# zhangmozhe/Deep-Exemplar-based-Video-Colorization

Hardware: AMD Instinct MI355X
Metric: colorized frames/sec/GPU at 216x384; correlation HBM GB/s vs roofline (higher is better)
Workload: dtype f32

## Files before the change

deep-exemplar-based-video-colorization_amd/csrc/conv_mfma.hip:

```cpp
#include "conv_kernel.h"
#include "conv_sk_kernel.h"
#include <algorithm>

#include "conv_wino_kernel.h"

static int virt_dim(int S, int up, int sub) {
    if (up == 2) return S * 2;
    if (sub == 2) return (S + 1) / 2;
    return S;
}

extern "C" int dvc_conv2d_out_hw(const DvcConvDesc* d, int32_t* OH, int32_t* OW) {
    DVC_REQUIRE(d, "dvc_conv2d_out_hw: null descriptor");
    int VH = virt_dim(d->H, d->in_up, d->in_sub), VW = virt_dim(d->W, d->in_up, d->in_sub);
    int ext = d->dil * (d->ksize - 1) + 1;
    *OH = (VH + 2 * d->pad - ext) / d->stride + 1;
    *OW = (VW + 2 * d->pad - ext) / d->stride + 1;
    return 0;
}

static int pick_tw(int OW) {
    int best = 32, best_w = cdiv(OW, 32) * 32;
    for (int tw : {16, 8}) {
        int wpad = cdiv(OW, tw) * tw;
// ... 758 lines not shown
#pragma unroll
    for (int o = 0; o < COUT; ++o) {
        float v = ((part[0][o][px] + part[1][o][px]) + (part[2][o][px] + part[3][o][px])) + (bias ? bias[o] : 0.f);
        y[((long)n * COUT + o) * HW + p] = apply_act(v, act, 0.f);
    }
}

extern "C" int dvc_conv1x1_small(const float* x, const float* w, const float* bias, int32_t N,
                                 int32_t Cin, int32_t HW, int32_t Cout, int32_t act, float* y,
                                 dvcStream stream) {
    DVC_REQUIRE(x && w && y, "dvc_conv1x1_small: null argument");
    DVC_REQUIRE(Cout >= 1 && Cout <= 4, "dvc_conv1x1_small: Cout must be 1..4");
    dim3 grid(cdiv(HW, 64), N);
    hipStream_t s = (hipStream_t)stream;
    switch (Cout) {
        case 1: hipLaunchKernelGGL(conv1x1_small_kernel<1>, grid, dim3(256), 0, s, x, w, bias, Cin, (long)HW, act, y); break;
        case 2: hipLaunchKernelGGL(conv1x1_small_kernel<2>, grid, dim3(256), 0, s, x, w, bias, Cin, (long)HW, act, y); break;
        case 3: hipLaunchKernelGGL(conv1x1_small_kernel<3>, grid, dim3(256), 0, s, x, w, bias, Cin, (long)HW, act, y); break;
        default: hipLaunchKernelGGL(conv1x1_small_kernel<4>, grid, dim3(256), 0, s, x, w, bias, Cin, (long)HW, act, y); break;
    }
    DVC_CHECK_LAUNCH("dvc_conv1x1_small");
    return 0;
}
```

deep-exemplar-based-video-colorization_amd/csrc/conv_wino_kernel.h:

```cpp
#pragma once
#include <type_traits>

#include "conv_kernel.h"

typedef float f32x4 __attribute__((ext_vector_type(4)));
typedef float f32x2 __attribute__((ext_vector_type(2)));

struct ConvWinoArgs {
    ConvKArgs k;
    int ss;
    int blk_y, blk_x;
    int gx, gy, gz;
    unsigned m_gx, m_gxy, m_cls, m_blkx, m_split;
    const float* x2;
    long x2_bs;
    int cinA, H2, W2, VH2, VW2, in_up2, in_sub2;
    float* pool;
    long pool_bs;
};
__host__ __device__ __forceinline__ unsigned wino_magic(long d) {
    return d > 1 ? (unsigned)(((1ULL << 32) + (unsigned long long)d - 1) / (unsigned long long)d) : 0u;
}
__device__ __forceinline__ int wino_div(int n, unsigned magic) { return magic ? (int)__umulhi((unsigned)n, magic) : n; }

// ... 41 lines not shown
#define WINO_S_ADD(D, A, B) asm volatile("v_add_f32 %0, %1, %2" : "=v"(D) : "v"(A), "v"(B))
#define WINO_S_SUB(D, A, B) asm volatile("v_sub_f32 %0, %1, %2" : "=v"(D) : "v"(A), "v"(B))

__device__ __forceinline__ int wino_stored_offset(int VH, int VW, int W, int in_up, int in_sub, int pad_mode, int vy, int vx) {
    int sy = map_virtual(vy, VH, pad_mode);
    int sx = map_virtual(vx, VW, pad_mode);
    if (sy < 0 || sx < 0) return -1;
    if (in_up == 2) {
        sy >>= 1;
        sx >>= 1;
    } else if (in_sub == 2) {
        sy <<= 1;
        sx <<= 1;
    }
    return sy * W + sx;
}

#define WINO_NBUF 3
__host__ __device__ constexpr int wino_xs_floats(int wm, int wn, int tr, int kc) {
    return ((kc * (2 * tr * wn + 2) * wino_pitch(tr) + 128 * wm * wn - 1) / (128 * wm * wn)) * (128 * wm * wn);
}
__host__ __device__ constexpr int wino_us_floats(int wm, int kc) { return wm * kc * 128 * 4; }

template <int WM, int WN, int TR, int KC, int VAR = 0, bool DUAL = false, class SA = ConvWinoArgs, bool UPZ = false>
__device__ __forceinline__ void conv_wino_body(const SA& s, const int wlog, float* const xsb, float* const usb) {
#if defined(__HIP_DEVICE_COMPILE__)
    const auto& a = s.k;
    constexpr int NPAIR = WM * WN;
    constexpr int NT = 128 * NPAIR;
    constexpr int TC = 32 / TR;
    constexpr int PR = 2 * TR * WN + 2;
    constexpr int PC = 2 * TC + 2;
    constexpr int PITCH = wino_pitch(TR);
    constexpr int plane = PR * PITCH;
    constexpr int EPT = (KC * plane + NT - 1) / NT;
    constexpr int C_XS = EPT * NT;
    static_assert(C_XS == wino_xs_floats(WM, WN, TR, KC), "LDS size helper out of step");
    constexpr int UQ = WM * KC * 128;
    static_assert(UQ * 4 == wino_us_floats(WM, KC), "LDS size helper out of step");
    static_assert(UQ % NT == 0, "whole staging instructions");
    static_assert(PITCH >= PC && PITCH % 2 == 0 && plane % 2 == 0 && KC % 4 == 0, "aligned patch rows, even K-steps per chunk");
    static_assert(2 * (PITCH / 2) + 1 < 256, "ds_read2_b64 offsets are 8 bits");
    constexpr int WPT = UQ / NT;
    constexpr int NI = EPT + WPT;
    static_assert(2 * NI < 64, "vmcnt is 6 bits");
    constexpr int KS = KC / 2;
    constexpr int NBUF = WINO_NBUF;
    constexpr int OOB = (int)0x80000000;
    static_assert(!UPZ || DUAL, "the zero-position form is built for the two-input launches");
    static_assert(NBUF * UQ * 4 >= 2 * NPAIR * 32 * 64, "the output exchange fits in the filter buffers");

    const int tid = threadIdx.x;
    const int lane = tid & 63, wave = __builtin_amdgcn_readfirstlane(tid >> 6);
    const int l31 = lane & 31, hi = lane >> 5;
    const int ph = wave / NPAIR, pair = wave % NPAIR;
    const int wm = pair / WN, wn = pair % WN;
    const int tr = l31 / TC, tc = l31 % TC;
    const int ss = s.ss;
    const int bz = wino_div(wlog, s.m_gxy), r_xy = wlog - bz * (s.gx * s.gy);
    const int by = wino_div(r_xy, s.m_gx), bx = r_xy - by * s.gx;
    const int per_cls = s.blk_y * s.blk_x;
    const int cls = wino_div(bx, s.m_cls), brem = bx - cls * per_cls;
    const int py = ss == 2 ? cls >> 1 : 0, px = ss == 2 ? cls & 1 : 0;
    const int tyb = wino_div(brem, s.m_blkx);
    const int ty0 = tyb * (TR * WN), tx0 = (brem - tyb * s.blk_x) * TC;
    const int b0 = by * WM;
    const int n = wino_div(bz, s.m_split), ksplit = bz - n * a.split;
    const int HWi = a.H * a.W;

    const int nchunks_all = a.Cin / KC;
    const int c_begin = ksplit * a.chunks_per_split;
    const int c_end = min(nchunks_all, c_begin + a.chunks_per_split);

// ... 68 lines not shown
    constexpr std::false_type ANY_INPUT{};

    const unsigned xlane =
        (unsigned)(size_t)(CONV_AS3 float*)xsb + (hi * plane + (2 * (wn * TR + tr) + ph) * PITCH + 2 * tc) * 4;
    const unsigned ulane = (unsigned)(size_t)(CONV_AS3 float*)usb + (((wm * KC + hi) * 4 + 2 * ph) * 32 + l31) * 16;

    constexpr bool BRANCH_FREE = VAR != 3;
    issue_x(c_begin, 0, ANY_INPUT);
    if (BRANCH_FREE) {
        issue(min(c_begin + 1, c_end - 1), 1, ANY_INPUT);
        issue(min(c_begin + 2, c_end - 1), 2, ANY_INPUT);
        asm volatile("s_waitcnt vmcnt(%0)" ::"n"(2 * NI) : "memory");
    } else {
        if (c_begin + 1 < c_end) issue(c_begin + 1, 1, ANY_INPUT);
        if (c_begin + 2 < c_end) issue(c_begin + 2, 2, ANY_INPUT);
        if (c_begin + 2 < c_end) asm volatile("s_waitcnt vmcnt(%0)" ::"n"(2 * NI) : "memory");
        else if (c_begin + 1 < c_end) asm volatile("s_waitcnt vmcnt(%0)" ::"n"(NI) : "memory");
        else asm volatile("s_waitcnt vmcnt(0)" ::: "memory");
    }
    __builtin_amdgcn_s_barrier();

    const float slope = a.act_slope_ptr ? *a.act_slope_ptr : a.act_slope;
    const long OHW = (long)a.OH * a.OW;
    const bool partial = a.split > 1;
    float* yb = partial ? a.part + ((long)ksplit * a.N + n) * a.Cout * OHW : a.y + (long)n * a.y_bs;
    const float* rb = (!partial && a.res) ? a.res + (long)n * a.res_bs : nullptr;

    auto run = [&](auto PHC) {
        constexpr int PH = decltype(PHC)::value;
        f32x4 D[2][3], U[2][2];
        f32x2 V03[2][2], V12[2][2];
        auto lo = [](const f32x4& v) { return __builtin_shufflevector(v, v, 0, 1); };
        auto hh = [](const f32x4& v) { return __builtin_shufflevector(v, v, 2, 3); };
        auto transform_a = [&](const f32x4 (&d)[3], f32x2 (&tl)[2], f32x2 (&th)[2], const bool row3_only = false) {
            if (VAR == 1) {
                if (PH == 0) {
                    WINO_S_SUB(tl[0].x, d[0].x, d[2].x); WINO_S_SUB(tl[0].y, d[0].y, d[2].y);
                    WINO_S_SUB(th[0].x, d[0].z, d[2].z); WINO_S_SUB(th[0].y, d[0].w, d[2].w);
                    WINO_S_ADD(tl[1].x, d[1].x, d[2].x); WINO_S_ADD(tl[1].y, d[1].y, d[2].y);
                    WINO_S_ADD(th[1].x, d[1].z, d[2].z); WINO_S_ADD(th[1].y, d[1].w, d[2].w);
                } else {
                    if (!row3_only) {
                        WINO_S_SUB(tl[0].x, d[1].x, d[0].x); WINO_S_SUB(tl[0].y, d[1].y, d[0].y);
                        WINO_S_SUB(th[0].x, d[1].z, d[0].z); WINO_S_SUB(th[0].y, d[1].w, d[0].w);
                    }
                    WINO_S_SUB(tl[1].x, d[0].x, d[2].x); WINO_S_SUB(tl[1].y, d[0].y, d[2].y);
                    WINO_S_SUB(th[1].x, d[0].z, d[2].z); WINO_S_SUB(th[1].y, d[0].w, d[2].w);
// ... 110 lines not shown
                    s1[j] = -m[j] - m[4 + j];
                }
            }
            o[0] = s0[0] + s0[1] + s0[2];
            o[1] = s0[1] - s0[2] - s0[3];
            o[2] = s1[0] + s1[1] + s1[2];
            o[3] = s1[1] - s1[2] - s1[3];
        };
        auto for8 = [&](auto f) {
            f(std::integral_constant<int, 0>{}); f(std::integral_constant<int, 1>{}); f(std::integral_constant<int, 2>{});
            f(std::integral_constant<int, 3>{}); f(std::integral_constant<int, 4>{}); f(std::integral_constant<int, 5>{});
            f(std::integral_constant<int, 6>{}); f(std::integral_constant<int, 7>{});
        };
        {
            float* mine = ex + (wave * 32) * 64 + lane;
            for8([&](auto IC) {
                constexpr int i = decltype(IC)::value;
                float o[4];
                partial_out(std::integral_constant<int, 8 * (1 - PH) + i>{}, o);
#pragma unroll
                for (int q = 0; q < 4; ++q) mine[(i * 4 + q) * 64] = o[q];
            });
        }
        __syncthreads();
        const float* theirs = ex + ((PH == 0 ? wave + NPAIR : wave - NPAIR) * 32) * 64 + lane;
        const int u0 = 2 * (ty0 + wn * TR + tr), x0 = 2 * (tx0 + tc);
        const int oy0 = ss * u0 + py, oy1 = ss * (u0 + 1) + py;
        const int ox0 = ss * x0 + px, ox1 = ss * (x0 + 1) + px;
        const bool okx0 = ox0 < a.OW, okx1 = ox1 < a.OW;
        const bool pairst = ss == 1 && okx1 && (a.OW & 1) == 0;
        const bool pool_here = !partial && s.pool;
        float* pb = pool_here ? s.pool + (long)n * s.pool_bs : nullptr;
        const long PHW = (long)(a.OH >> 1) * (a.OW >> 1);
        for8([&](auto IC) {
            constexpr int i = decltype(IC)::value;
            constexpr int r = 8 * PH + i;
            float o[4];
            partial_out(std::integral_constant<int, r>{}, o);
#pragma unroll
            for (int q = 0; q < 4; ++q) {
                const float t = theirs[(i * 4 + q) * 64];
                o[q] = PH == 0 ? o[q] + t : t + o[q];
            }
            const int co = (b0 + wm) * 32 + (r & 3) + 8 * (r >> 2) + 4 * hi;
            const float bias = (!partial && a.bias) ? a.bias[co] : 0.f;
            float pooled = 0.f;
#pragma unroll
            for (int p = 0; p < 2; ++p) {
                const int oy = p ? oy1 : oy0;
                if (oy >= a.OH) continue;
                const long row = (long)co * OHW + (long)oy * a.OW;
                float v0 = o[2 * p] + bias, v1 = o[2 * p + 1] + bias;
                if (rb) {
                    if (okx0) v0 += rb[row + ox0];
                    if (okx1) v1 += rb[row + ox1];
                }
                if (!partial) {
                    v0 = apply_act(v0, a.act, slope);
                    v1 = apply_act(v1, a.act, slope);
                }
                if (pool_here) {
                    const float m = fmaxf(v0, v1);
                    pooled = p ? fmaxf(pooled, m) : m;
                    if (p && okx1) pb[(long)co * PHW + (long)(oy0 >> 1) * (a.OW >> 1) + (ox0 >> 1)] = pooled;
                    if (!a.y) continue;
                }
                if (pairst && VAR == 2) {
                    union { float2 f; unsigned long long u; } cv;
                    cv.f = make_float2(v0, v1);
                    __hip_atomic_store(reinterpret_cast<unsigned long long*>(yb + row + ox0), cv.u, __ATOMIC_RELAXED, __HIP_MEMORY_SCOPE_AGENT);
                } else if (pairst) {
                    *reinterpret_cast<float2*>(yb + row + ox0) = make_float2(v0, v1);
                } else {
                    if (okx0) yb[row + ox0] = v0;
                    if (okx1) yb[row + ox1] = v1;
                }
            }
        });
    };
    if (ph) run(std::integral_constant<int, 1>{});
    else run(std::integral_constant<int, 0>{});
#endif
}

template <int WM, int WN, int TR, int KC, int VAR = 0, bool DUAL = false, bool UPZ = false>
__global__ __launch_bounds__(128 * WM * WN) __attribute__((amdgpu_waves_per_eu(2, 2))) void conv_wino_kernel(ConvWinoArgs s) {
    __shared__ __attribute__((aligned(16))) float xsb[WINO_NBUF * wino_xs_floats(WM, WN, TR, KC)];
    __shared__ __attribute__((aligned(16))) float usb[WINO_NBUF * wino_us_floats(WM, KC)];
    const int G = s.gx * s.gy * s.gz;
    const int xq = G / 8, xr = G % 8, xcd = blockIdx.x % 8, xi = blockIdx.x / 8;
    const int wlog = (xcd < xr ? xcd * (xq + 1) : xr * (xq + 1) + (xcd - xr) * xq) + xi;
    conv_wino_body<WM, WN, TR, KC, VAR, DUAL, ConvWinoArgs, UPZ>(s, wlog, xsb, usb);
}

#define WINO_GROUP_MAX 4
struct ConvWinoGroupArgs {
    ConvWinoArgs item[WINO_GROUP_MAX];
    int per_xcd[WINO_GROUP_MAX + 1];
    int tr[WINO_GROUP_MAX];
    int n;
};
typedef __attribute__((address_space(4))) ConvWinoArgs ConvWinoArgsK;
template <int WM, int WN, int KC>
__global__ __launch_bounds__(128 * WM * WN) __attribute__((amdgpu_waves_per_eu(2, 2))) void conv_wino_group_kernel(ConvWinoGroupArgs g) {
    constexpr int XS = wino_xs_floats(WM, WN, 1, KC) > wino_xs_floats(WM, WN, 8, KC) ? wino_xs_floats(WM, WN, 1, KC) : wino_xs_floats(WM, WN, 8, KC);
    static_assert(XS >= wino_xs_floats(WM, WN, 2, KC) && XS >= wino_xs_floats(WM, WN, 4, KC), "largest patch buffer");
#if defined(__HIP_DEVICE_COMPILE__)
    __shared__ __attribute__((aligned(16))) float xsb[WINO_NBUF * XS];
    __shared__ __attribute__((aligned(16))) float usb[WINO_NBUF * wino_us_floats(WM, KC)];
    const int xcd = blockIdx.x % 8, xi = blockIdx.x / 8;
    int it = 0, base = 0, q = g.per_xcd[1], tr = g.tr[0];
#pragma unroll
    for (int i = 1; i < WINO_GROUP_MAX; ++i)
        if (i < g.n && xi >= g.per_xcd[i]) {
            it = i;
// ... 56 lines not shown
}

template <int WM, int WN, int KC>
static void conv_wino_launch_shape_dual(int tr, bool upz, dim3 grid, hipStream_t st, const ConvWinoArgs& s) {
    constexpr int NT = 128 * WM * WN;
    if (upz) {
        switch (tr) {
            case 1: hipLaunchKernelGGL((conv_wino_kernel<WM, WN, 1, KC, 0, true, true>), grid, dim3(NT), 0, st, s); break;
            case 2: hipLaunchKernelGGL((conv_wino_kernel<WM, WN, 2, KC, 0, true, true>), grid, dim3(NT), 0, st, s); break;
            case 4: hipLaunchKernelGGL((conv_wino_kernel<WM, WN, 4, KC, 0, true, true>), grid, dim3(NT), 0, st, s); break;
            default: hipLaunchKernelGGL((conv_wino_kernel<WM, WN, 8, KC, 0, true, true>), grid, dim3(NT), 0, st, s); break;
        }
        return;
    }
    switch (tr) {
        case 1: hipLaunchKernelGGL((conv_wino_kernel<WM, WN, 1, KC, 0, true>), grid, dim3(NT), 0, st, s); break;
        case 2: hipLaunchKernelGGL((conv_wino_kernel<WM, WN, 2, KC, 0, true>), grid, dim3(NT), 0, st, s); break;
        case 4: hipLaunchKernelGGL((conv_wino_kernel<WM, WN, 4, KC, 0, true>), grid, dim3(NT), 0, st, s); break;
        default: hipLaunchKernelGGL((conv_wino_kernel<WM, WN, 8, KC, 0, true>), grid, dim3(NT), 0, st, s); break;
    }
}

void conv_wino_launch_m1_dual(int tr, bool upz, dim3 grid, hipStream_t st, const ConvWinoArgs& s);
void conv_wino_launch_m4(int tr, dim3 grid, hipStream_t st, const ConvWinoArgs& s);
void conv_wino_launch_m2(int tr, dim3 grid, hipStream_t st, const ConvWinoArgs& s);
void conv_wino_launch_m1(int tr, dim3 grid, hipStream_t st, const ConvWinoArgs& s);
void conv_wino_launch_m0(int tr, dim3 grid, hipStream_t st, const ConvWinoArgs& s);
void conv_wino_launch_group_m1(dim3 grid, hipStream_t st, const ConvWinoGroupArgs& g);
```

deep-exemplar-based-video-colorization_amd/csrc/conv_wino_m1.hip:

```cpp
#include "conv_wino_kernel.h"

void conv_wino_launch_m1(int tr, dim3 grid, hipStream_t st, const ConvWinoArgs& s) {
    conv_wino_launch_shape<2, 1, 4>(tr, grid, st, s);
}

void conv_wino_launch_m1_dual(int tr, bool upz, dim3 grid, hipStream_t st, const ConvWinoArgs& s) {
    conv_wino_launch_shape_dual<2, 1, 4>(tr, upz, grid, st, s);
}
```

deep-exemplar-based-video-colorization_amd/dvc_amd/_lib.py:

```python
import ctypes
import os

_HERE = os.path.dirname(os.path.abspath(__file__))
DEBUG_BUILD = os.environ.get("DVC_DEBUG_LIB", "0") == "1"
LIB_PATH = os.path.join(_HERE, "libdvc_hip_debug.so" if DEBUG_BUILD else "libdvc_hip.so")
ABI_VERSION = 20

c_float_p = ctypes.c_void_p
c_i32 = ctypes.c_int32
c_i64 = ctypes.c_int64


class DvcConvDesc(ctypes.Structure):
    _fields_ = [
        ("N", c_i32), ("Cin", c_i32), ("H", c_i32), ("W", c_i32),
        ("Cout", c_i32), ("ksize", c_i32), ("stride", c_i32), ("dil", c_i32),
        ("pad", c_i32), ("pad_mode", c_i32), ("in_up", c_i32), ("in_sub", c_i32),
        ("act", c_i32), ("act_slope", ctypes.c_float), ("in_prelu", c_i32), ("cfg", c_i32), ("split_k", c_i32),
        ("x_batch_stride", c_i64), ("y_batch_stride", c_i64), ("res_batch_stride", c_i64),
        ("flags", c_i32), ("w_batch_stride", c_i64),
    ]


class DvcConvGroupItem(ctypes.Structure):
# ... 17 lines not shown
_VP = ctypes.c_void_p
SIGNATURES = {
    "dvc_abi_version": (ctypes.c_int, []),
    "dvc_last_error": (ctypes.c_char_p, []),
    "dvc_conv2d_out_hw": (ctypes.c_int, [ctypes.POINTER(DvcConvDesc), ctypes.POINTER(c_i32), ctypes.POINTER(c_i32)]),
    "dvc_conv2d": (ctypes.c_int, [ctypes.POINTER(DvcConvDesc), _VP, _VP, _VP, _VP, _VP, _VP, _VP, _VP, _VP, _VP,
                                  ctypes.c_size_t, _VP]),
    "dvc_winograd_weight_floats": (ctypes.c_size_t, [c_i32, c_i32]),
    "dvc_winograd_pack_weight": (ctypes.c_int, [_VP, c_i32, c_i32, _VP, _VP]),
    "dvc_conv2d_winograd_split": (ctypes.c_int, [ctypes.POINTER(DvcConvDesc), ctypes.c_size_t, ctypes.POINTER(c_i32),
                                                ctypes.POINTER(c_i32)]),
    "dvc_conv2d_winograd": (ctypes.c_int, [ctypes.POINTER(DvcConvDesc), _VP, _VP, _VP, _VP, _VP, _VP, _VP,
                                           ctypes.c_size_t, _VP]),
    "dvc_conv2d_winograd_pool": (ctypes.c_int, [ctypes.POINTER(DvcConvDesc), _VP, _VP, _VP, _VP, _VP, _VP, c_i64, _VP,
                                                ctypes.c_size_t, _VP]),
    "dvc_conv2d_winograd_dual": (ctypes.c_int, [ctypes.POINTER(DvcConvDesc), ctypes.POINTER(DvcConvDesc), _VP, _VP, _VP, _VP, _VP,
                                                _VP, _VP, ctypes.c_size_t, _VP]),
    "dvc_conv2d_ws_eligible": (ctypes.c_int, [ctypes.POINTER(DvcConvDesc)]),
    "dvc_conv2d_ws_pack_weight": (ctypes.c_int, [_VP, c_i32, c_i32, _VP, _VP]),
    "dvc_conv2d_ws": (ctypes.c_int, [ctypes.POINTER(DvcConvDesc), _VP, _VP, _VP, _VP, _VP, _VP]),
    "dvc_conv2d_winograd_group": (ctypes.c_int, [ctypes.POINTER(DvcConvGroupItem), c_i32, _VP]),
    "dvc_instnorm_apply_group": (ctypes.c_int, [ctypes.POINTER(DvcInstNormItem), c_i32, _VP]),
    "dvc_conv1x1_small": (ctypes.c_int, [_VP, _VP, _VP, c_i32, c_i32, c_i32, c_i32, c_i32, _VP, _VP]),
    "dvc_instnorm_stats": (ctypes.c_int, [_VP, c_i32, c_i32, c_i32, c_i64, ctypes.c_float, _VP, _VP, _VP, _VP]),
    "dvc_affine_act": (ctypes.c_int, [_VP, _VP, _VP, _VP, _VP, c_i32, c_i32, c_i32, c_i32, c_i32, c_i32,
                                      c_i64, c_i64, c_i64, _VP, _VP]),
    "dvc_instnorm_apply": (ctypes.c_int, [_VP, _VP, _VP, _VP, ctypes.c_float, c_i32, c_i32, c_i32, c_i32, c_i32,
                                          c_i32, c_i32, c_i64, c_i64, c_i64, _VP, _VP, _VP, _VP, c_i32, _VP, _VP]),
    "dvc_cx_prepare": (ctypes.c_int, [_VP, _VP, c_i32, c_i32, c_i32, c_i32, ctypes.c_float, _VP, _VP, _VP, _VP]),
    "dvc_cx_rows": (ctypes.c_int, [_VP, c_i32, c_i64, c_i64, c_i32, c_i32, ctypes.c_float, _VP, _VP, _VP, _VP, _VP, _VP]),
    "dvc_cx_colmax": (ctypes.c_int, [_VP, c_i32, c_i64, c_i64, _VP, _VP, c_i32, c_i32, c_i32, ctypes.c_float, _VP, _VP, _VP]),
    "dvc_cx_finish": (ctypes.c_int, [_VP, c_i32, c_i32, _VP, _VP, _VP]),
    "dvc_cx_rows_tq": (ctypes.c_int, [_VP, c_i32, c_i64, c_i64, c_i64, _VP, _VP, _VP, c_i32, c_i32, c_i32, ctypes.c_float, _VP, _VP,
                                      _VP]),
    "dvc_cx_ds": (ctypes.c_int, [_VP, c_i32, c_i64, c_i64, c_i64, _VP, _VP, _VP, _VP, _VP, _VP, _VP, _VP, _VP, ctypes.c_float, c_i32,
                                 c_i32, c_i32, c_i32, c_i32, ctypes.c_float, _VP, _VP, _VP]),
    "dvc_cx_normalize_bwd": (ctypes.c_int, [_VP, _VP, _VP, c_i32, c_i32, c_i32, ctypes.c_float, _VP, _VP]),
    "dvc_instnorm_apply_partials": (ctypes.c_int, [_VP, c_i32, _VP, c_i32, ctypes.c_float, _VP, _VP, _VP, _VP, ctypes.c_float,
                                                   c_i32, c_i32, c_i32, c_i32, c_i32, c_i32, c_i32, c_i64, c_i64, _VP, _VP, _VP,
                                                   _VP, c_i32, _VP, _VP]),
    "dvc_maxpool2x2": (ctypes.c_int, [_VP, c_i32, c_i32, c_i32, _VP, _VP]),
    "dvc_avgpool2x2": (ctypes.c_int, [_VP, c_i32, c_i32, c_i32, _VP, _VP]),
    "dvc_avgpool4x4": (ctypes.c_int, [_VP, c_i32, c_i32, c_i32, _VP, _VP]),
    "dvc_upsample_nearest": (ctypes.c_int, [_VP, c_i32, c_i32, c_i32, c_i32, _VP, _VP]),
    "dvc_channel_l2norm": (ctypes.c_int, [_VP, c_i32, c_i32, c_i32, ctypes.c_float, _VP, _VP]),
    "dvc_channel_l2norm_multi": (ctypes.c_int, [_VP, _VP, _VP, _VP, c_i32, c_i32, ctypes.c_float, _VP]),
# ... 113 lines not shown
```

deep-exemplar-based-video-colorization_amd/dvc_amd/graph.py:

```python
import torch

from . import nets, ops


def _epoch():
    return (nets.pack_epoch(),) + ops.launch_epoch()


class CapturedSequence:

    def __init__(self, fn, stream):
        self.workspaces = {}
        self.graph = torch.cuda.CUDAGraph()
        stream.wait_stream(torch.cuda.current_stream())
        with ops.workspace_scope(self.workspaces):
            with torch.cuda.stream(stream):
                fn()
            stream.synchronize()
            self.epoch = _epoch()
            with torch.cuda.graph(self.graph, stream=stream):
                self.out = fn()
        if _epoch() != self.epoch:
            raise RuntimeError("dvc_amd.graph: a weight was packed during stream capture (warm-up did not cover the sequence)")

    def stale(self):
        return _epoch() != self.epoch

    def replay(self):
        self.graph.replay()
# ... 1 lines not shown
```

deep-exemplar-based-video-colorization_amd/dvc_amd/nets.py:

```python
import torch
import torch.nn as nn
from torch.autograd.function import once_differentiable

from . import arch, ops

_VGG_MEAN_BGR = (0.40760392, 0.45795686, 0.48501961)


_pack_epoch = 0


def pack_epoch():
    return _pack_epoch


class _PackCache:

    def __init__(self):
        self._d = {}

    def get(self, key, param, fn):
        params = param if isinstance(param, tuple) else (param,)
        tag = tuple((p.data_ptr(), _version_of(p), str(p.device)) for p in params)
        param = params[0]
# ... 671 lines not shown
        return self._cache.get(key, self._mod(key).weight, lambda w: w.detach().reshape(-1).contiguous())

    def _out_weight(self):
        out = self._mod(arch.CVN_OUT["key"])
        return self._cache.get("conv10_ab", out.weight, lambda w: w.detach().reshape(w.shape[0], -1).contiguous())

    def _dual_pack(self, cA, cB):
        mA, mB = self._mod(cA["key"]), self._mod(cB["key"])
        u = self._cache.get(cA["key"] + ":dual", (mA.weight, mB.weight), lambda ws: torch.cat(
            (ops.pack_winograd_weight(ws[0]), ops.pack_winograd_weight(ws[1])), dim=1).contiguous())
        b = self._cache.get(cA["key"] + ":dualbias", (mA.bias, mB.bias), lambda bs: (bs[0].detach() + bs[1].detach()).contiguous())
        return u, b

    def _dual_ok(self, cA, cB, shapeA, shapeB):
        if not ops.dual_conv_enabled():
            return False
        (N, CA, HA, WA), (_, CB, HB, WB) = shapeA, shapeB
        upA = 2 if cA["pre"] == "up" else 1
        if cA["cout"] % 64 or cB["cout"] != cA["cout"] or CA % 8 or CB % 8:
            return False
        return (ops.winograd_selected(N, CA, HA, WA, cA["cout"], dil=cA["dil"], pad=cA["dil"], in_up=upA, layer="cvn." + cA["key"])
                and ops.winograd_selected(N, CB, HB, WB, cB["cout"], dil=cB["dil"], pad=cB["dil"], layer="cvn." + cB["key"]))

    def prepare(self):
        for c in arch.CVN_CONVS:
            _prepack(self._cache, c["key"], self._mod(c["key"]))
            if c["pre"] == "norm_ss":
                self._ss_weight(c["ss"])
        self._out_weight()
        if ops.conv_algo() != "direct" and ops.dual_conv_enabled():
            G = arch.CVN_GRAPH
            for key, skip in G.dual.items():
                self._dual_pack(G.by_key[key], G.by_key[skip])

    def forward(self, x):
        if self.training and torch.is_grad_enabled() and (x.requires_grad or any(p.requires_grad for p in self.parameters())):
            return self._forward_with_grad(x)
        _check_input(x, "ColorVidNet")
        return self._forward(x)

    def _forward_with_grad(self, x):
        if not x.is_cuda:
            _check_input(x, "ColorVidNet")
        if x.dtype != torch.float32:
            raise TypeError(f"ColorVidNet: the training path takes a float32 input (got {x.dtype})")
        named = list(self.named_parameters())
# ... 96 lines not shown
                            ops.record_layer("cvn." + cc_["key"], src_.shape[1], cc_["cout"], src_.shape[2], src_.shape[3], dil=cc_["dil"],
                                             in_up=2 if cc_["pre"] == "up" else 1, dual=c["key"])
                    acts[c["dst"]] = ops.conv2d_winograd_dual(srcA, srcB, u, b, dil=c["dil"], in_upA=2 if c["pre"] == "up" else 1,
                                                              act=act_map[c["act"]], act_slope=0.2)
                    produced(c["dst"])
                    continue
                convE = self._mod(e["key"])
                acts[e["dst"]] = ops.conv3x3(srcB, convE.weight, _packs(self._cache, e["key"], convE.weight), convE.bias.detach(),
                                             dil=e["dil"], act=act_map[e["act"]], act_slope=0.2, layer="cvn." + e["key"])
            conv = self._mod(c["key"])
            kw = dict(dil=c["dil"], act=act_map[c["act"]], act_slope=0.2)
            pre = c["pre"]
            src = acts[c["src"]]
            if pre == "norm":
                src = norm_of(c["src"])
            elif pre == "norm_ss":
                src = norm_of(c["src"], c["ss"])
            elif pre == "up":
                src = norm_of(c["src"])
                kw["in_up"] = 2
            if c["add"] is not None:
                kw["residual"] = acts[c["add"]]
            dst = c["dst"]
            acts[dst] = ops.conv3x3(src, conv.weight, _packs(self._cache, c["key"], conv.weight), conv.bias.detach(),
                                    defer_reduce=dst in G.norm_only and saved is None, layer="cvn." + c["key"], **kw)
            produced(dst)
        out = self._mod(arch.CVN_OUT["key"])
        if saved is not None:
            saved.update((a, acts[a]) for a in G.saved_acts)
            saved["x"] = x
        return ops.conv1x1_small(acts[arch.CVN_OUT["src"]], self._out_weight(), out.bias.detach(), act=ops.ACT_TANH128)
```

deep-exemplar-based-video-colorization_amd/dvc_amd/ops.py:

```python
import ctypes
import os as _os
import sys
from typing import NamedTuple

import torch

from . import _lib
from ._lib import DvcConvDesc, DvcConvGroupItem, DvcInstNormItem

ACT_NONE, ACT_RELU, ACT_PRELU, ACT_LEAKY, ACT_TANH128 = 0, 1, 2, 3, 4
PAD_ZERO, PAD_REFLECT = 0, 1
EPS64 = sys.float_info.epsilon


def _p(t):
    return None if t is None else ctypes.c_void_p(t.data_ptr())


def _pv(t):
    return None if t is None else t.data_ptr()


_raw_stream = getattr(torch._C, "_cuda_getCurrentRawStream", None)
_raw_device = getattr(torch._C, "_cuda_getDevice", None)
# ... 113 lines not shown
def _flag_functions(var, getter, setter):
    g = globals()

    def get():
        return g[var]

    def set_(flag=True):
        g[var] = bool(flag)
    get.__name__ = get.__qualname__ = getter
    set_.__name__ = set_.__qualname__ = setter
    return get, set_


for _sw in _SWITCHES:
    globals()[_sw.var] = _sw.parse(_os.environ.get(_sw.env, _sw.default) if _sw.env else _sw.default)
    if _sw.setter:
        globals()[_sw.getter], globals()[_sw.setter] = _flag_functions(_sw.var, _sw.getter, _sw.setter)
del _sw


def launch_epoch():
    g = globals()
    return tuple(g[sw.getter]() for sw in _SWITCHES if sw.launch)


def autotune_enabled():
    return _autotune


def set_autotune(flag=True):
    global _autotune
    _autotune = bool(flag)
    if _autotune:
        _load_tuned()


def conv_algo():
    return _conv_algo


def set_conv_algo(algo):
    global _conv_algo
    if algo not in ("auto", "speed", "direct", "winograd"):
        raise ValueError("conv algo must be 'auto', 'speed', 'direct' or 'winograd'")
    _conv_algo = algo

# ... 482 lines not shown
        S, ipl = _winograd_split(lib, d, ws.numel())
        need = (S * N * Cout * OH * OW * 4 + 255) // 256 * 256 if S > 1 else 0
        room = ws.numel() - off
        S2, ipl2 = _winograd_split(lib, d, max(room, 0))
        if need > room or S2 != S or ipl < N or ipl2 < N:
            return [single(it_, j) for j, it_ in enumerate(items)]
        defer = it.get("defer_reduce", False) and _fuse_reduce and S > 1 and _may_defer(act, OH, OW)
        if defer:
            d.flags |= DEFER_REDUCE
        out = None if defer else torch.empty((N, Cout, OH, OW), device=dev, dtype=torch.float32)
        a = arr[i]
        a.d = d
        a.x, a.u_packed, a.bias, a.act_slope_ptr, a.residual = x.data_ptr(), u.data_ptr(), _pv(bias), _pv(act_slope_t), None
        a.y = ws.data_ptr() + off if out is None else out.data_ptr()
        a.workspace, a.workspace_bytes = ws.data_ptr() + off, room
        meta.append((out, S, (N, Cout, OH, OW), bias, act, act_slope, act_slope_t, off, u))
        off += need
    generation = _bump_generation(ws)
    _lib.check(lib.dvc_conv2d_winograd_group(arr, n, _stream()), "dvc_conv2d_winograd_group")
    return [out if out is not None else ConvPartials(ws, S, shape, bias, act, act_slope, act_slope_t, generation, dev, offset=o)
            for (out, S, shape, bias, act, act_slope, act_slope_t, o, _u) in meta]


def conv1x1_small(x, w, bias, act=ACT_NONE):
    lib = _lib.load()
    _need_all(x=x, w=w, bias=bias)
    N, Cin, H, W = x.shape
    Cout = w.shape[0]
    y = torch.empty((N, Cout, H, W), device=x.device, dtype=torch.float32)
    _lib.check(lib.dvc_conv1x1_small(_p(x), _p(w), _p(bias), N, Cin, H * W, Cout, act, _p(y), _stream()),
               "dvc_conv1x1_small")
    return y


def instnorm_stats(x, eps=1e-5, chan_scale=None):
    lib = _lib.load()
    _need_all(x=x, chan_scale=chan_scale)
    N, C, H, W = x.shape
    scale = torch.empty(N * C, device=x.device, dtype=torch.float32)
    shift = torch.empty(N * C, device=x.device, dtype=torch.float32)
    _lib.check(lib.dvc_instnorm_stats(_p(x), N, C, H * W, 0, float(eps), _p(chan_scale), _p(scale), _p(shift),
                                      _stream()), "dvc_instnorm_stats")
    return scale, shift


def affine_act(x, scale, shift, *, residual=None, slope_t=None, up=1, rpad=0, out=None, out_batch_stride=0):
# ... 608 lines not shown
```

include/dvc_hip.h:

```cpp
#ifndef DVC_HIP_H
#define DVC_HIP_H

#include <stddef.h>
#include <stdint.h>

#ifdef __cplusplus
extern "C" {
#endif

#pragma GCC visibility push(default)

typedef void* dvcStream;

#define DVC_ABI_VERSION 20

int dvc_abi_version(void);
const char* dvc_last_error(void);

enum { DVC_ACT_NONE = 0, DVC_ACT_RELU = 1, DVC_ACT_PRELU = 2, DVC_ACT_LEAKY = 3, DVC_ACT_TANH128 = 4 };
enum { DVC_PAD_ZERO = 0, DVC_PAD_REFLECT = 1 };

typedef struct DvcConvDesc {
    int32_t N, Cin, H, W;
    int32_t Cout;
// ... 45 lines not shown
                             const float* act_slope_ptr , float* y,
                             void* workspace , size_t workspace_bytes, dvcStream stream);

int dvc_conv2d_ws_eligible(const DvcConvDesc* d);
int dvc_conv2d_ws_pack_weight(const float* w, int32_t Cout, int32_t Cin, float* u_packed, dvcStream stream);
int dvc_conv2d_ws(const DvcConvDesc* d, const float* x, const float* u_packed, const float* bias ,
                  const float* act_slope_ptr , float* y, dvcStream stream);

typedef struct DvcConvGroupItem {
    DvcConvDesc d;
    const float* x;
    const float* u_packed;
    const float* bias;
    const float* act_slope_ptr;
    const float* residual;
    float* y;
    void* workspace;
    size_t workspace_bytes;
} DvcConvGroupItem;
int dvc_conv2d_winograd_group(const DvcConvGroupItem* items, int32_t n_items, dvcStream stream);

int dvc_conv1x1_small(const float* x, const float* w, const float* bias, int32_t N, int32_t Cin,
                      int32_t HW, int32_t Cout, int32_t act, float* y, dvcStream stream);

int dvc_instnorm_stats(const float* x, int32_t N, int32_t C, int32_t HW, int64_t x_batch_stride,
                       float eps, const float* chan_scale, float* scale, float* shift,
                       dvcStream stream);

int dvc_affine_act(const float* x, const float* scale, const float* shift, const float* residual,
                   const float* slope_ptr, int32_t N, int32_t C, int32_t H, int32_t W, int32_t up,
                   int32_t rpad, int64_t x_batch_stride, int64_t res_batch_stride,
                   int64_t y_batch_stride, float* y, dvcStream stream);

int dvc_instnorm_apply(const float* x, const float* residual , const float* slope_ptr ,
                       const float* chan_scale , float eps, int32_t N, int32_t C, int32_t H,
                       int32_t W, int32_t up, int32_t sub, int32_t rpad, int64_t x_batch_stride,
                       int64_t res_batch_stride, int64_t y_batch_stride, float* y,
                       float* scale_out, float* shift_out,
                       const float* chan_scale2 , int32_t sub2, float* y2 ,
                       dvcStream stream);
int dvc_instnorm_apply_partials(const float* part, int32_t S, const float* bias, int32_t act, float act_slope,
                                const float* act_slope_ptr, const float* residual, const float* slope_ptr,
                                const float* chan_scale, float eps, int32_t N, int32_t C, int32_t H, int32_t W, int32_t up,
                                int32_t sub, int32_t rpad, int64_t res_batch_stride, int64_t y_batch_stride, float* y,
                                float* scale_out, float* shift_out, const float* chan_scale2, int32_t sub2, float* y2,
                                dvcStream stream);
// ... 169 lines not shown
```

Baseline: 437.7.

## Fuse final 1x1 output head into last Winograd 3x3 conv epilogue

Adds a HEAD variant of the Winograd conv kernel for the last colorization-net conv (Cout=128). Its epilogue applies bias and activation, then computes the 1x1 head projection (up to 4 outputs) from LDS-resident tiles. Each of the two 64-channel halves writes partial sums to a workspace, and a small finish kernel adds them with the head bias and tanh. This avoids writing and rereading the full 128-channel activation and the separate conv1x1_small launch. The cost is extra LDS use, added barriers in the epilogue, and one extra small kernel.

After: 440.3 (median of 6 runs). No clear change (+0.6%).

```diff
diff --git a/deep-exemplar-based-video-colorization_amd/csrc/conv_mfma.hip b/deep-exemplar-based-video-colorization_amd/csrc/conv_mfma.hip
--- a/deep-exemplar-based-video-colorization_amd/csrc/conv_mfma.hip
+++ b/deep-exemplar-based-video-colorization_amd/csrc/conv_mfma.hip
@@ -804,3 +804,80 @@
     DVC_CHECK_LAUNCH("dvc_conv1x1_small");
     return 0;
 }
+
+template <int V>
+__global__ __launch_bounds__(256) void conv1x1_head_finish_kernel(const float* __restrict__ s0, const float* __restrict__ s1,
+                                                                  const float* __restrict__ bias, int HC, long HW, long total,
+                                                                  int act, float* __restrict__ y) {
+    const long e = ((long)blockIdx.x * 256 + threadIdx.x) * V;
+    if (e >= total) return;
+    const float b = bias ? bias[(e / HW) % HC] : 0.f;
+    if (V == 4) {
+        const float4 p = *reinterpret_cast<const float4*>(s0 + e), q = *reinterpret_cast<const float4*>(s1 + e);
+        *reinterpret_cast<float4*>(y + e) = make_float4(apply_act((p.x + q.x) + b, act, 0.f), apply_act((p.y + q.y) + b, act, 0.f),
+                                                        apply_act((p.z + q.z) + b, act, 0.f), apply_act((p.w + q.w) + b, act, 0.f));
+    } else {
+        y[e] = apply_act((s0[e] + s1[e]) + b, act, 0.f);
+    }
+}
+
+static bool wino_head_plan_ok(const DvcConvDesc* d, size_t workspace_bytes, int head_cout) {
+    if (d->Cout != 128 || d->dil != 1 || head_cout < 1 || head_cout > 4 || (d->flags & DVC_CONV_DEFER_REDUCE)) return false;
+    int32_t OH, OW;
+    dvc_conv2d_out_hw(d, &OH, &OW);
+    if (OH <= 0 || OW <= 0 || (size_t)2 * d->N * head_cout * OH * OW * sizeof(float) > workspace_bytes) return false;
+    int m, tr, S;
+    wino_plan(d, OH, OW, workspace_bytes > 0, workspace_bytes, &m, &tr, &S);
+    if (m != 2) return false;
+    const int nch = d->Cin / kWinoShapes[m].kc;
+    return cdiv(nch, cdiv(nch, S)) == 1 && wino_images_per_launch(d, OH, OW, m, tr, 1, workspace_bytes) > 0;
+}
+
+extern "C" int dvc_conv2d_winograd_head_fusable(const DvcConvDesc* d, size_t workspace_bytes, int32_t head_cout, int32_t* fusable) {
+    DVC_REQUIRE(d && fusable, "dvc_conv2d_winograd_head_fusable: null argument");
+    if (int rc = wino_check_desc(d)) return rc;
+    *fusable = wino_head_plan_ok(d, workspace_bytes, head_cout) ? 1 : 0;
+    return 0;
+}
+
+extern "C" int dvc_conv2d_winograd_head(const DvcConvDesc* d, const float* x, const float* u_packed, const float* bias,
+                                        const float* act_slope_ptr, const float* head_w, const float* head_bias,
+                                        int32_t head_cout, int32_t head_act, float* y, void* workspace, size_t workspace_bytes,
+                                        dvcStream stream) {
+    DVC_REQUIRE(d && x && u_packed && head_w && y && workspace, "dvc_conv2d_winograd_head: null argument");
+    if (int rc = wino_check_desc(d)) return rc;
+    DVC_REQUIRE(wino_head_plan_ok(d, workspace_bytes, head_cout),
+                "dvc_conv2d_winograd_head: not a layer this form takes (see dvc_conv2d_winograd_head_fusable)");
+    DVC_REQUIRE((reinterpret_cast<uintptr_t>(workspace) & 15) == 0, "dvc_conv2d_winograd_head: workspace must be 16-byte aligned");
+    int32_t OH, OW;
+    dvc_conv2d_out_hw(d, &OH, &OW);
+    const long OHW = (long)OH * OW, col = (long)d->N * head_cout * OHW;
+    float* part = reinterpret_cast<float*>(workspace);
+    ConvWinoArgs s;
+    int best_m = -1, best_tr = 1, group = 0;
+    if (int rc = wino_setup(d, nullptr, x, nullptr, u_packed, bias, act_slope_ptr, nullptr, nullptr, workspace, workspace_bytes, part,
+                            col, s, &best_m, &best_tr, &group))
+        return rc;
+    DVC_REQUIRE(best_m == 2 && s.k.split == 1, "dvc_conv2d_winograd_head: plan changed between the check and the setup");
+    s.x2 = head_w;
+    s.H2 = head_cout;
+    hipStream_t st = (hipStream_t)stream;
+    for (int n0 = 0; n0 < d->N; n0 += group) {
+        const int NB = std::min(group, d->N - n0);
+        s.k.N = NB;
+        s.k.x = x + (long)n0 * s.k.x_bs;
+        s.pool = part + (long)n0 * head_cout * OHW;
+        const dim3 grid = wino_finish_grid(s, NB);
+        conv_wino_launch_m1_head(best_tr, grid, st, s);
+        DVC_CHECK_LAUNCH("dvc_conv2d_winograd_head");
+    }
+    const bool v4 = OHW % 4 == 0 && (reinterpret_cast<uintptr_t>(y) & 15) == 0;
+    if (v4)
+        hipLaunchKernelGGL(conv1x1_head_finish_kernel<4>, dim3((unsigned)((col / 4 + 255) / 256)), dim3(256), 0, st, part, part + col,
+                           head_bias, head_cout, OHW, col, head_act, y);
+    else
+        hipLaunchKernelGGL(conv1x1_head_finish_kernel<1>, dim3((unsigned)((col + 255) / 256)), dim3(256), 0, st, part, part + col,
+                           head_bias, head_cout, OHW, col, head_act, y);
+    DVC_CHECK_LAUNCH("dvc_conv2d_winograd_head(finish)");
+    return 0;
+}
diff --git a/deep-exemplar-based-video-colorization_amd/csrc/conv_wino_kernel.h b/deep-exemplar-based-video-colorization_amd/csrc/conv_wino_kernel.h
--- a/deep-exemplar-based-video-colorization_amd/csrc/conv_wino_kernel.h
+++ b/deep-exemplar-based-video-colorization_amd/csrc/conv_wino_kernel.h
@@ -87,7 +87,7 @@
 }
 __host__ __device__ constexpr int wino_us_floats(int wm, int kc) { return wm * kc * 128 * 4; }
 
-template <int WM, int WN, int TR, int KC, int VAR = 0, bool DUAL = false, class SA = ConvWinoArgs, bool UPZ = false>
+template <int WM, int WN, int TR, int KC, int VAR = 0, bool DUAL = false, class SA = ConvWinoArgs, bool UPZ = false, bool HEAD = false>
 __device__ __forceinline__ void conv_wino_body(const SA& s, const int wlog, float* const xsb, float* const usb) {
 #if defined(__HIP_DEVICE_COMPILE__)
     const auto& a = s.k;
@@ -114,6 +114,9 @@
     constexpr int OOB = (int)0x80000000;
     static_assert(!UPZ || DUAL, "the zero-position form is built for the two-input launches");
     static_assert(NBUF * UQ * 4 >= 2 * NPAIR * 32 * 64, "the output exchange fits in the filter buffers");
+    static_assert(!HEAD || (WM == 2 && WN == 1 && !DUAL && VAR == 0), "the head epilogue is built for the 64 x 32 shape");
+    static_assert(!HEAD || NBUF * UQ * 4 >= 2 * NPAIR * 32 * 64 + 4 * 128 + NPAIR * 128,
+                  "... and pair 1's sums and the head's weights fit behind the exchange");
 
     const int tid = threadIdx.x;
     const int lane = tid & 63, wave = __builtin_amdgcn_readfirstlane(tid >> 6);
@@ -228,7 +231,7 @@
 
     const float slope = a.act_slope_ptr ? *a.act_slope_ptr : a.act_slope;
     const long OHW = (long)a.OH * a.OW;
-    const bool partial = a.split > 1;
+    const bool partial = !HEAD && a.split > 1;
     float* yb = partial ? a.part + ((long)ksplit * a.N + n) * a.Cout * OHW : a.y + (long)n * a.y_bs;
     const float* rb = (!partial && a.res) ? a.res + (long)n * a.res_bs : nullptr;
 
@@ -385,8 +388,12 @@
                 for (int q = 0; q < 4; ++q) mine[(i * 4 + q) * 64] = o[q];
             });
         }
+        if constexpr (HEAD) {
+            const int e = PH * 64 + lane, oo = e & 3;
+            ex[2 * NPAIR * 32 * 64 + 4 * 128 + pair * 128 + e] = s.x2[(oo < s.H2 ? oo : 0) * a.Cout + (b0 + wm) * 32 + (e >> 2)];
+        }
         __syncthreads();
-        const float* theirs = ex + ((PH == 0 ? wave + NPAIR : wave - NPAIR) * 32) * 64 + lane;
+        float* const theirs = ex + ((PH == 0 ? wave + NPAIR : wave - NPAIR) * 32) * 64 + lane;
         const int u0 = 2 * (ty0 + wn * TR + tr), x0 = 2 * (tx0 + tc);
         const int oy0 = ss * u0 + py, oy1 = ss * (u0 + 1) + py;
         const int ox0 = ss * x0 + px, ox1 = ss * (x0 + 1) + px;
@@ -407,6 +414,11 @@
             }
             const int co = (b0 + wm) * 32 + (r & 3) + 8 * (r >> 2) + 4 * hi;
             const float bias = (!partial && a.bias) ? a.bias[co] : 0.f;
+            if constexpr (HEAD) {
+#pragma unroll
+                for (int q = 0; q < 4; ++q) theirs[(i * 4 + q) * 64] = apply_act(o[q] + bias, a.act, slope);
+                return;
+            }
             float pooled = 0.f;
 #pragma unroll
             for (int p = 0; p < 2; ++p) {
@@ -440,20 +452,53 @@
                 }
             }
         });
+        if constexpr (HEAD) {
+            __syncthreads();
+            const int hc = s.H2, q = 2 * PH + hi;
+            const float* grp = ex + (pair * 32) * 64 + q * 64 + l31;
+            const f32x4* hwl = reinterpret_cast<const f32x4*>(ex + 2 * NPAIR * 32 * 64 + 4 * 128 + pair * 128);
+            float acc[4] = {0.f, 0.f, 0.f, 0.f};
+#pragma unroll 1
+            for (int b = 0; b < 8; ++b) {
+                const float* g4 = grp + ((1 - (b >> 2)) * NPAIR * 32 + 16 * ((b >> 1) & 1)) * 64 + (b & 1) * 32;
+#pragma unroll
+                for (int j = 0; j < 4; ++j) {
+                    const float v = g4[j * 4 * 64];
+                    const f32x4 w4 = hwl[4 * b + j];
+                    acc[0] = fmaf(v, w4.x, acc[0]);
+                    acc[1] = fmaf(v, w4.y, acc[1]);
+                    acc[2] = fmaf(v, w4.z, acc[2]);
+                    acc[3] = fmaf(v, w4.w, acc[3]);
+                }
+            }
+            float* comb = ex + 2 * NPAIR * 32 * 64 + PH * 64 + lane;
+            if (wm == 1) {
+#pragma unroll
+                for (int oo = 0; oo < 4; ++oo) comb[oo * 128] = acc[oo];
+            }
+            __syncthreads();
+            const int oy = PH ? oy1 : oy0, ox = hi ? ox1 : ox0;
+            if (wm == 0 && oy < a.OH && ox < a.OW) {
+                float* sp = s.pool + (long)by * s.pool_bs + (long)n * hc * OHW + (long)oy * a.OW + ox;
+#pragma unroll
+                for (int oo = 0; oo < 4; ++oo)
+                    if (oo < hc) sp[oo * OHW] = acc[oo] + comb[oo * 128];
+            }
+        }
     };
     if (ph) run(std::integral_constant<int, 1>{});
     else run(std::integral_constant<int, 0>{});
 #endif
 }
 
-template <int WM, int WN, int TR, int KC, int VAR = 0, bool DUAL = false, bool UPZ = false>
+template <int WM, int WN, int TR, int KC, int VAR = 0, bool DUAL = false, bool UPZ = false, bool HEAD = false>
 __global__ __launch_bounds__(128 * WM * WN) __attribute__((amdgpu_waves_per_eu(2, 2))) void conv_wino_kernel(ConvWinoArgs s) {
     __shared__ __attribute__((aligned(16))) float xsb[WINO_NBUF * wino_xs_floats(WM, WN, TR, KC)];
     __shared__ __attribute__((aligned(16))) float usb[WINO_NBUF * wino_us_floats(WM, KC)];
     const int G = s.gx * s.gy * s.gz;
     const int xq = G / 8, xr = G % 8, xcd = blockIdx.x % 8, xi = blockIdx.x / 8;
     const int wlog = (xcd < xr ? xcd * (xq + 1) : xr * (xq + 1) + (xcd - xr) * xq) + xi;
-    conv_wino_body<WM, WN, TR, KC, VAR, DUAL, ConvWinoArgs, UPZ>(s, wlog, xsb, usb);
+    conv_wino_body<WM, WN, TR, KC, VAR, DUAL, ConvWinoArgs, UPZ, HEAD>(s, wlog, xsb, usb);
 }
 
 #define WINO_GROUP_MAX 4
@@ -556,6 +601,7 @@
 }
 
 void conv_wino_launch_m1_dual(int tr, bool upz, dim3 grid, hipStream_t st, const ConvWinoArgs& s);
+void conv_wino_launch_m1_head(int tr, dim3 grid, hipStream_t st, const ConvWinoArgs& s);
 void conv_wino_launch_m4(int tr, dim3 grid, hipStream_t st, const ConvWinoArgs& s);
 void conv_wino_launch_m2(int tr, dim3 grid, hipStream_t st, const ConvWinoArgs& s);
 void conv_wino_launch_m1(int tr, dim3 grid, hipStream_t st, const ConvWinoArgs& s);
diff --git a/deep-exemplar-based-video-colorization_amd/csrc/conv_wino_m1.hip b/deep-exemplar-based-video-colorization_amd/csrc/conv_wino_m1.hip
--- a/deep-exemplar-based-video-colorization_amd/csrc/conv_wino_m1.hip
+++ b/deep-exemplar-based-video-colorization_amd/csrc/conv_wino_m1.hip
@@ -7,3 +7,12 @@
 void conv_wino_launch_m1_dual(int tr, bool upz, dim3 grid, hipStream_t st, const ConvWinoArgs& s) {
     conv_wino_launch_shape_dual<2, 1, 4>(tr, upz, grid, st, s);
 }
+
+void conv_wino_launch_m1_head(int tr, dim3 grid, hipStream_t st, const ConvWinoArgs& s) {
+    switch (tr) {
+        case 1: hipLaunchKernelGGL((conv_wino_kernel<2, 1, 1, 4, 0, false, false, true>), grid, dim3(256), 0, st, s); break;
+        case 2: hipLaunchKernelGGL((conv_wino_kernel<2, 1, 2, 4, 0, false, false, true>), grid, dim3(256), 0, st, s); break;
+        case 4: hipLaunchKernelGGL((conv_wino_kernel<2, 1, 4, 4, 0, false, false, true>), grid, dim3(256), 0, st, s); break;
+        default: hipLaunchKernelGGL((conv_wino_kernel<2, 1, 8, 4, 0, false, false, true>), grid, dim3(256), 0, st, s); break;
+    }
+}
diff --git a/deep-exemplar-based-video-colorization_amd/dvc_amd/_lib.py b/deep-exemplar-based-video-colorization_amd/dvc_amd/_lib.py
--- a/deep-exemplar-based-video-colorization_amd/dvc_amd/_lib.py
+++ b/deep-exemplar-based-video-colorization_amd/dvc_amd/_lib.py
@@ -63,6 +63,9 @@
     "dvc_conv2d_winograd_group": (ctypes.c_int, [ctypes.POINTER(DvcConvGroupItem), c_i32, _VP]),
     "dvc_instnorm_apply_group": (ctypes.c_int, [ctypes.POINTER(DvcInstNormItem), c_i32, _VP]),
     "dvc_conv1x1_small": (ctypes.c_int, [_VP, _VP, _VP, c_i32, c_i32, c_i32, c_i32, c_i32, _VP, _VP]),
+    "dvc_conv2d_winograd_head_fusable": (ctypes.c_int, [ctypes.POINTER(DvcConvDesc), ctypes.c_size_t, c_i32, ctypes.POINTER(c_i32)]),
+    "dvc_conv2d_winograd_head": (ctypes.c_int, [ctypes.POINTER(DvcConvDesc), _VP, _VP, _VP, _VP, _VP, _VP, c_i32, c_i32, _VP, _VP,
+                                                ctypes.c_size_t, _VP]),
     "dvc_instnorm_stats": (ctypes.c_int, [_VP, c_i32, c_i32, c_i32, c_i64, ctypes.c_float, _VP, _VP, _VP, _VP]),
     "dvc_affine_act": (ctypes.c_int, [_VP, _VP, _VP, _VP, _VP, c_i32, c_i32, c_i32, c_i32, c_i32, c_i32,
                                       c_i64, c_i64, c_i64, _VP, _VP]),
diff --git a/deep-exemplar-based-video-colorization_amd/dvc_amd/graph.py b/deep-exemplar-based-video-colorization_amd/dvc_amd/graph.py
--- a/deep-exemplar-based-video-colorization_amd/dvc_amd/graph.py
+++ b/deep-exemplar-based-video-colorization_amd/dvc_amd/graph.py
@@ -4,7 +4,7 @@
 
 
 def _epoch():
-    return (nets.pack_epoch(),) + ops.launch_epoch()
+    return ((nets.pack_epoch(), ops.head_fusion()),) + ops.launch_epoch()
 
 
 class CapturedSequence:
diff --git a/deep-exemplar-based-video-colorization_amd/dvc_amd/nets.py b/deep-exemplar-based-video-colorization_amd/dvc_amd/nets.py
--- a/deep-exemplar-based-video-colorization_amd/dvc_amd/nets.py
+++ b/deep-exemplar-based-video-colorization_amd/dvc_amd/nets.py
@@ -717,6 +717,13 @@
         return (ops.winograd_selected(N, CA, HA, WA, cA["cout"], dil=cA["dil"], pad=cA["dil"], in_up=upA, layer="cvn." + cA["key"])
                 and ops.winograd_selected(N, CB, HB, WB, cB["cout"], dil=cB["dil"], pad=cB["dil"], layer="cvn." + cB["key"]))
 
+    def _head_ok(self, c, shape):
+        N, Cin, H, W = shape
+        if not ops.head_fusion() or c["pre"] is not None or c["add"] is not None or c["dil"] != 1 or c is not arch.CVN_CONVS[-1]:
+            return False
+        return (ops.winograd_selected(N, Cin, H, W, c["cout"], layer="cvn." + c["key"])
+                and ops.winograd_head_fusable(N, Cin, H, W, c["cout"], arch.CVN_OUT["cout"]))
+
     def prepare(self):
         for c in arch.CVN_CONVS:
             _prepack(self._cache, c["key"], self._mod(c["key"]))
@@ -859,6 +866,13 @@
             if c["add"] is not None:
                 kw["residual"] = acts[c["add"]]
             dst = c["dst"]
+            if dst == arch.CVN_OUT["src"] and saved is None and self._head_ok(c, src.shape):
+                if ops.layer_record is not None:
+                    ops.record_layer("cvn." + c["key"], src.shape[1], c["cout"], src.shape[2], src.shape[3], head=arch.CVN_OUT["key"])
+                out = self._mod(arch.CVN_OUT["key"])
+                return ops.conv2d_winograd_head(src, _packs(self._cache, c["key"], conv.weight)("winograd"), conv.bias.detach(),
+                                                self._out_weight(), out.bias.detach(), act=kw["act"], act_slope=0.2,
+                                                head_act=ops.ACT_TANH128)
             acts[dst] = ops.conv3x3(src, conv.weight, _packs(self._cache, c["key"], conv.weight), conv.bias.detach(),
                                     defer_reduce=dst in G.norm_only and saved is None, layer="cvn." + c["key"], **kw)
             produced(dst)
diff --git a/deep-exemplar-based-video-colorization_amd/dvc_amd/ops.py b/deep-exemplar-based-video-colorization_amd/dvc_amd/ops.py
--- a/deep-exemplar-based-video-colorization_amd/dvc_amd/ops.py
+++ b/deep-exemplar-based-video-colorization_amd/dvc_amd/ops.py
@@ -159,6 +159,10 @@
 def launch_epoch():
     g = globals()
     return tuple(g[sw.getter]() for sw in _SWITCHES if sw.launch)
+
+
+_fuse_head = _on_unless_0(_os.environ.get("DVC_FUSE_HEAD", "1"))
+head_fusion, set_head_fusion = _flag_functions("_fuse_head", "head_fusion", "set_head_fusion")
 
 
 def autotune_enabled():
@@ -687,6 +691,43 @@
             for (out, S, shape, bias, act, act_slope, act_slope_t, o, _u) in meta]
 
 
+_head_fusable = {}
+
+
+def winograd_head_fusable(N, Cin, H, W, Cout, head_cout):
+    if not winograd_eligible(Cin, Cout) or Cout != 128 or not 1 <= head_cout <= 4:
+        return False
+    key = (N, Cin, H, W, Cout, head_cout, _plan_flags(N))
+    got = _head_fusable.get(key)
+    if got is None:
+        ok = ctypes.c_int32(0)
+        d = _conv_desc(N, Cin, H, W, Cout, flags=key[-1])
+        _lib.check(_lib.load().dvc_conv2d_winograd_head_fusable(ctypes.byref(d), CONV_WORKSPACE_BYTES, head_cout, ctypes.byref(ok)),
+                   "dvc_conv2d_winograd_head_fusable")
+        got = _head_fusable[key] = bool(ok.value)
+    return got
+
+
+def conv2d_winograd_head(x, u_packed, bias, head_w, head_bias, *, act=ACT_NONE, act_slope=0.0, act_slope_t=None, head_act=ACT_NONE):
+    lib = _lib.load()
+    _need_all(x=x, u_packed=u_packed, bias=bias, act_slope=act_slope_t, head_w=head_w, head_bias=head_bias)
+    N, Cin, H, W = x.shape
+    assert u_packed.dim() == 5 and u_packed.shape[1] == Cin and tuple(u_packed.shape[2:]) == (4, 32, 4), u_packed.shape
+    Cout = u_packed.shape[0] * 32
+    hc = head_w.shape[0]
+    assert head_w.dim() == 2 and head_w.shape[1] == Cout and head_w.is_contiguous(), head_w.shape
+    d = _conv_desc(N, Cin, H, W, Cout, act=act, act_slope=act_slope, flags=_plan_flags(N))
+    if conv_record is not None:
+        conv_record.append(_record_conv(d, affine=False, in_prelu=False, residual=False, algo="winograd-head"))
+    ws = _workspace(x.device, CONV_WORKSPACE_BYTES, "conv")
+    _bump_generation(ws)
+    y = torch.empty((N, hc, H, W), device=x.device, dtype=torch.float32)
+    _lib.check(lib.dvc_conv2d_winograd_head(ctypes.byref(d), _p(x), _p(u_packed), _p(bias), _p(act_slope_t), _p(head_w), _p(head_bias),
+                                            hc, head_act, _p(y), ctypes.c_void_p(ws.data_ptr()), ws.numel(), _stream()),
+               "dvc_conv2d_winograd_head")
+    return y
+
+
 def conv1x1_small(x, w, bias, act=ACT_NONE):
     lib = _lib.load()
     _need_all(x=x, w=w, bias=bias)
diff --git a/include/dvc_hip.h b/include/dvc_hip.h
--- a/include/dvc_hip.h
+++ b/include/dvc_hip.h
@@ -91,6 +91,11 @@
 
 int dvc_conv1x1_small(const float* x, const float* w, const float* bias, int32_t N, int32_t Cin,
                       int32_t HW, int32_t Cout, int32_t act, float* y, dvcStream stream);
+int dvc_conv2d_winograd_head_fusable(const DvcConvDesc* d, size_t workspace_bytes, int32_t head_cout, int32_t* fusable);
+int dvc_conv2d_winograd_head(const DvcConvDesc* d, const float* x, const float* u_packed, const float* bias ,
+                             const float* act_slope_ptr , const float* head_w,
+                             const float* head_bias , int32_t head_cout, int32_t head_act, float* y,
+                             void* workspace, size_t workspace_bytes, dvcStream stream);
 
 int dvc_instnorm_stats(const float* x, int32_t N, int32_t C, int32_t HW, int64_t x_batch_stride,
                        float eps, const float* chan_scale, float* scale, float* shift,
```
